# NVlabs/FoundationPose

Measured on NVIDIA H100. Metric: pose-hypotheses/sec at 640x480 RGB-D, 252 hyp, 5 refine iters, higher is better.
Workload: dtype f16

## Files before the change

foundationpose_b200/csrc/fp_api_ops.cu:

```cuda
#include "../../include/fpose.h"
#include "fp_common.cuh"
#include "fp_attn.cuh"
#include "fp_crop.cuh"
#include "fp_gemm.cuh"

#include <vector>

namespace fp {
const char* get_last_error();
int prof_collect(int kind, double* total_ms, double* total_work, int* launches);
}

extern "C" {

const char* fp_last_error(void) { return fp::get_last_error(); }

unsigned long long fp_launch_count(void) { return fp::launch_count(); }

int fp_prof_enable(int on) {
  fp::g_prof_on = on != 0;
  return 0;
}

int fp_prof_collect(int kind, double* total_ms, double* total_work, int* launches) {
  if (!total_ms || !total_work || !launches) {
    fp::set_last_error("fp_prof_collect: null output");
    return -1;
  }
  return fp::prof_collect(kind, total_ms, total_work, launches);
}

int fp_op_build_meshlets(int V, int F, const float* pos, const int* faces, int* info, int* face_of_tri_out,
                         float* meshlets_out) {
  try {
    if (!pos || !faces || !info || V <= 0 || F <= 0) {
      fp::set_last_error("fp_op_build_meshlets: bad argument");
      return -1;
    }
    for (int i = 0; i < 3 * F; ++i)
      if (faces[i] < 0 || faces[i] >= V) {
        fp::set_last_error("fp_op_build_meshlets: face index out of range");
        return -1;
      }
    std::vector<float> nrm((size_t)V * 3, 0.f), att((size_t)V * 3, 0.f);
    fp::MeshHost mh;
    int rc = fp::build_mesh_host(V, F, pos, nrm.data(), att.data(), 3, faces, mh);
    if (rc) return rc;
    int max_t = 0, max_v = 0, total = 0;
    for (const fp::Meshlet& m : mh.meshlets) {
      max_t = m.n_tris > max_t ? m.n_tris : max_t;
      max_v = m.n_verts > max_v ? m.n_verts : max_v;
      total += m.n_tris;
      for (int t = 0; t < m.n_tris; ++t) {
        const uint2 tr = mh.ml_tris[m.tri_off + t];
        for (int k = 0; k < 3; ++k) {
          const int slot = (tr.x >> (8 * k)) & 255;
          if (slot >= m.n_verts || mh.ml_verts[m.vert_off + slot] != faces[3 * tr.y + k]) {
            fp::set_last_error("fp_op_build_meshlets: meshlet triangle does not map back to its face");
            return -4;
          }
          const float* q = pos + 3 * faces[3 * tr.y + k];
          const float dx = q[0] - m.cx, dy = q[1] - m.cy, dz = q[2] - m.cz;
          if (dx * dx + dy * dy + dz * dz > m.r * m.r * 1.0001f + 1e-12f) {
            fp::set_last_error("fp_op_build_meshlets: vertex outside the meshlet's bounding sphere");
            return -4;
          }
        }
        if (face_of_tri_out) face_of_tri_out[m.tri_off + t] = (int)tr.y;
      }
    }
    if (meshlets_out)
      for (size_t i = 0; i < mh.meshlets.size(); ++i) {
        const fp::Meshlet& m = mh.meshlets[i];
        const float rec[8] = {m.cx, m.cy, m.cz, m.r, m.ax, m.ay, m.az, m.cutoff};
        for (int k = 0; k < 8; ++k) meshlets_out[8 * i + k] = rec[k];
      }
    info[0] = (int)mh.meshlets.size();
    info[1] = mh.closed;
    info[2] = mh.front_sign;
    info[3] = max_t;
    info[4] = max_v;
    info[5] = total;
    return 0;
  } catch (...) {
    fp::set_last_error("fp_op_build_meshlets: exception");
    return -3;
  }
}

int fp_op_attention(const void* qkv, void* out, int B, int impl, void* stream) {
  if (!qkv || !out) {
    fp::set_last_error("fp_op_attention: null argument");
    return -1;
  }
  fp::AttnParams ap;
  ap.qkv = reinterpret_cast<const __half*>(qkv);
  ap.ld = 1536;
  ap.q_off = 0;
  ap.k_off = 512;
  ap.v_off = 1024;
  ap.group_col_stride = 0;
  ap.n_groups = 1;
  ap.out = reinterpret_cast<__half*>(out);
  ap.ld_out = 512;
  ap.out_group_stride = 0;
  ap.B = B;
  ap.T = 400;
  ap.n_heads = 4;
  ap.scale = 0.08838834764831845f;
  cudaStream_t st = reinterpret_cast<cudaStream_t>(stream);
  (void)impl;
  return fp::attn_tc_launch(ap, st);
}

static fp::GemmLayer to_gemm_layer(const fp_gemm_layer_t* l) {
  fp::GemmLayer L;
  L.kind = l->kind;
  L.n_img = l->n_img;
  L.Hin = l->Hin;
  L.Win = l->Win;
  L.Cin = l->Cin;
  L.Cout = l->Cout;
  L.in = l->in;
  L.w = l->w;
  L.bias = l->bias;
  L.res = l->res;
  L.res_ld = l->res_ld;
  L.out = l->out;
  L.out_ld = l->out_ld;
  L.out_split = l->out_split;
  L.post_add = l->post_add;
  L.relu = l->relu;
  return L;
}

int fp_op_gemm_layer(const fp_gemm_layer_t* l, void* stream) {
  if (!l) {
    fp::set_last_error("fp_op_gemm_layer: null layer");
    return -1;
  }
  return fp::gemm_layer_launch(to_gemm_layer(l), reinterpret_cast<cudaStream_t>(stream));
}

int fp_op_gemm_tile_n(const fp_gemm_layer_t* l, int* tile_n) {
  if (!l || !tile_n) {
    fp::set_last_error("fp_op_gemm_tile_n: null argument");
    return -1;
  }
  return fp::gemm_layer_tile_n(to_gemm_layer(l), tile_n);
}

}
```

foundationpose_b200/csrc/fp_gemm.cu:

```cuda
#include "fp_gemm.cuh"

#include <stdarg.h>
#include <stdlib.h>
#include <string.h>

#include <mutex>
#include <vector>

#include "fp_common.cuh"
#include "fp_wgmma.cuh"

namespace fp {

static std::atomic<unsigned long long> g_launch_count{0};
static thread_local bool t_capturing = false;
void note_launches(int n) {
  if (!t_capturing) g_launch_count.fetch_add((unsigned long long)n, std::memory_order_relaxed);
}
unsigned long long launch_count() { return g_launch_count.load(std::memory_order_relaxed); }
void set_capturing(bool on) { t_capturing = on; }

std::atomic<bool> g_prof_on{false};
static std::mutex g_prof_mu;

struct ProfRec {
  cudaEvent_t e0, e1;
  double work;
  int kind;
};
static std::vector<ProfRec> g_prof_recs;

void prof_mark_begin(int kind, double work, cudaStream_t stream) {
  if (!g_prof_on) return;
  ProfRec r;
  r.kind = kind;
  r.work = work;
  cudaEventCreate(&r.e0);
  cudaEventCreate(&r.e1);
  cudaEventRecord(r.e0, stream);
  std::lock_guard<std::mutex> lk(g_prof_mu);
  g_prof_recs.push_back(r);
}
void prof_mark_end(cudaStream_t stream) {
  if (!g_prof_on) return;
  std::lock_guard<std::mutex> lk(g_prof_mu);
  if (g_prof_recs.empty()) return;
  cudaEventRecord(g_prof_recs.back().e1, stream);
}
int prof_collect(int kind, double* total_ms, double* total_work, int* launches) {
  FP_CUDA_OK(cudaDeviceSynchronize());
  std::lock_guard<std::mutex> lk(g_prof_mu);
  double ms = 0, work = 0;
  int n = 0;
  std::vector<ProfRec> keep;
  for (auto& r : g_prof_recs) {
    if (r.kind != kind) {
      keep.push_back(r);
      continue;
    }
    float t = 0.f;
    cudaEventElapsedTime(&t, r.e0, r.e1);
    ms += t;
    work += r.work;
    ++n;
    cudaEventDestroy(r.e0);
    cudaEventDestroy(r.e1);
  }
  g_prof_recs.swap(keep);
  *total_ms = ms;
  *total_work = work;
  *launches = n;
  return 0;
}

static thread_local char t_last_error[1024] = "";
void set_last_error(const char* fmt, ...) {
  va_list ap;
  va_start(ap, fmt);
  vsnprintf(t_last_error, sizeof(t_last_error), fmt, ap);
  va_end(ap);
}
const char* get_last_error() { return t_last_error; }

static thread_local int t_pdl_skip = 0;
void pdl_skip_next() { t_pdl_skip = 1; }

bool pdl_enabled() {
  if (t_pdl_skip) {
    t_pdl_skip = 0;
    return false;
  }
  static int on = -1;
  if (on < 0) {
    const char* e = getenv("FPOSE_PDL");
    on = (e && e[0] == '0') ? 0 : 1;
  }
  return on != 0;
}

struct GemmParams {
  int lg_bw, lg_bh;
  int bw, bh, bn;
  int tiles_w, tiles_h, tiles_n, n_tiles_n, total_tiles;
  int num_kb, chunks_per_tap;
  int dim_w, dim_h, dim_n;
  short tap_off[9][5];
  int Ho, Wo, n_img, Cout;
  const float* bias;
  int has_res;
  int odim_h, odim_n;
  int out_split;
  const float* post_add;
  int relu;
  double alg_flops;
};

constexpr int kBlockM = 128;
constexpr int kBlockK = 64;
constexpr int kABytes = kBlockM * kBlockK * 2;
constexpr int kTileThreads = 384;
constexpr int kSlabBytes = kBlockM * 64 * 2;
constexpr int kSmemOptIn = 232448;

constexpr int kWideSlabs = 2;
constexpr int kWideProducerRegs = 40;
constexpr int kWideConsumerRegs = 232;
template <int BN>
struct TileCfg {
  static constexpr int kBBytes = BN * kBlockK * 2;
  static constexpr int kStageBytes = kABytes + kBBytes;
  static constexpr int kSlabs = BN > 128 ? kWideSlabs : BN / 64;
  static constexpr int kPasses = BN / 64 / kSlabs;
  static constexpr int kStagingBytes = kSlabs * kSlabBytes;
  static constexpr int kRing = kSmemOptIn - kStagingBytes - 1024  - 256 ;
  static constexpr int kStages = (kRing / kStageBytes) > 8 ? 8 : (kRing / kStageBytes);
  static constexpr int kSmemBytes = kStages * kStageBytes + kStagingBytes + 1024 + 256;
  static_assert(kSmemBytes <= kSmemOptIn, "tile configuration exceeds the 227 KB opt-in shared memory");
  static_assert(kPasses * kSlabs * 64 == BN, "the epilogue passes must cover the tile's channels");
};

template <int BN>
__global__ void __launch_bounds__(kTileThreads, 1)
    gemm_tile_kernel(const __grid_constant__ CUtensorMap map_a, const __grid_constant__ CUtensorMap map_b,
                     const __grid_constant__ CUtensorMap map_out, const __grid_constant__ CUtensorMap map_res,
                     const __grid_constant__ GemmParams p) {
  using Cfg = TileCfg<BN>;
  constexpr int S = Cfg::kStages;
  constexpr int NSLAB = Cfg::kSlabs;
  constexpr int JP = BN / 8 / Cfg::kPasses;
  extern __shared__ uint8_t smem_raw[];
  uint8_t* smem = reinterpret_cast<uint8_t*>((reinterpret_cast<uintptr_t>(smem_raw) + 1023) & ~uintptr_t(1023));
  uint8_t* staging = smem + S * Cfg::kStageBytes;
  uint64_t* bars = reinterpret_cast<uint64_t*>(staging + Cfg::kStagingBytes);
  uint64_t* full = bars;
  uint64_t* empty = bars + S;
  uint64_t* res_full = bars + 2 * S;

  const int m_tiles = p.tiles_w * p.tiles_h * p.tiles_n;
  const int total = m_tiles * p.n_tiles_n;

  if (threadIdx.x == 0) {
    tma_prefetch_desc(&map_a);
    tma_prefetch_desc(&map_b);
    tma_prefetch_desc(&map_out);
    if (p.has_res) tma_prefetch_desc(&map_res);
    for (int s = 0; s < S; ++s) {
      mbar_init(&full[s], 1);
      mbar_init(&empty[s], 256);
    }
    mbar_init(res_full, 1);
    mbar_fence_init();
  }
  __syncthreads();
  pdl_trigger();
  pdl_wait();

  auto decode = [&](int t, int& n_tile, int& tw, int& th, int& tn) {
    n_tile = t % p.n_tiles_n;
    const int m_tile = t / p.n_tiles_n;
    tw = m_tile % p.tiles_w;
    th = (m_tile / p.tiles_w) % p.tiles_h;
    tn = m_tile / (p.tiles_w * p.tiles_h);
  };

  if (threadIdx.x < 128) {
    if constexpr (BN > 128) regs_release<kWideProducerRegs>();
    if (threadIdx.x == 0) {
      int stage = 0, phase = 0;
      for (int t = blockIdx.x; t < total; t += gridDim.x) {
        int n_tile, tw, th, tn;
        decode(t, n_tile, tw, th, tn);
        int base[5] = {0, 0, 0, 0, 0};
        base[p.dim_w] += tw * p.bw;
        if (p.dim_h >= 0) base[p.dim_h] += th * p.bh;
        if (p.dim_n >= 0) base[p.dim_n] += tn * p.bn;
        int tap = 0, chunk = 0;
        for (int kb = 0; kb < p.num_kb; ++kb) {
          mbar_wait(&empty[stage], phase ^ 1);
          uint8_t* sa = smem + stage * Cfg::kStageBytes;
          mbar_expect_tx(&full[stage], Cfg::kStageBytes);
          tma_load_5d(&map_a, &full[stage], sa, base[0] + p.tap_off[tap][0] + chunk * kBlockK, base[1] + p.tap_off[tap][1],
                      base[2] + p.tap_off[tap][2], base[3] + p.tap_off[tap][3], base[4] + p.tap_off[tap][4]);
          tma_load_2d(&map_b, &full[stage], sa + kABytes, kb * kBlockK, n_tile * BN);
          if (++chunk == p.chunks_per_tap) {
            chunk = 0;
            ++tap;
          }
          if (++stage == S) {
            stage = 0;
            phase ^= 1;
          }
        }
      }
    }
    return;
  }

  if constexpr (BN > 128) regs_acquire<kWideConsumerRegs>();
  const int ct = threadIdx.x - 128;
  const int cw = ct >> 7;
  const int lane = threadIdx.x & 31;
  const int r0 = 64 * cw + 16 * ((ct >> 5) & 3) + (lane >> 2);
  const int cq = 2 * (lane & 3);
  const bool leader = (ct == 0);
  float acc[BN / 2];
#pragma unroll
  for (int i = 0; i < BN / 2; ++i) acc[i] = 0.f;
  int stage = 0, phase = 0, it = 0;
  for (int t = blockIdx.x; t < total; t += gridDim.x, ++it) {
    int n_tile, tw, th, tn;
    decode(t, n_tile, tw, th, tn);
    const int n0 = tn * p.bn;
    int n_o0 = n0, coff = 0;
    if (p.out_split > 0) {
      n_o0 = n0 % p.out_split;
      coff = (n0 / p.out_split) * p.Cout;
    }
    int oc[5] = {0, 0, 0, 0, 0}, rc[5] = {0, 0, 0, 0, 0};
    oc[1] = rc[1] = tw * p.bw;
    if (p.odim_h >= 0) oc[p.odim_h] = rc[p.odim_h] = th * p.bh;
    if (p.odim_n >= 0) {
      oc[p.odim_n] = n_o0;
      rc[p.odim_n] = n0;
    }
    if (leader) asm volatile("cp.async.bulk.wait_group.read 0;" ::: "memory");
    asm volatile("bar.sync 1, 256;" ::: "memory");
    if (leader && p.has_res) {
      mbar_expect_tx(res_full, NSLAB * kSlabBytes);
      for (int s = 0; s < NSLAB; ++s)
        tma_load_5d(&map_res, res_full, staging + s * kSlabBytes, n_tile * BN + s * 64, rc[1], rc[2], rc[3], rc[4]);
    }

    int prev = -1;
    for (int kb = 0; kb < p.num_kb; ++kb) {
      mbar_wait(&full[stage], phase);
      const uint32_t sa = smem_u32(smem + stage * Cfg::kStageBytes);
      const uint64_t da = gmma_desc_sw128(sa + (uint32_t)cw * 8192u);
      const uint64_t db = gmma_desc_sw128(sa + kABytes);
      wgmma_fence();
#pragma unroll
      for (int k = 0; k < kBlockK / 16; ++k)
        Wgmma<BN>::ss(acc, da + (uint64_t)(2 * k), db + (uint64_t)(2 * k), (kb > 0 || k > 0) ? 1u : 0u);
      wgmma_commit();
      if (prev >= 0) {
        wgmma_wait<1>();
        mbar_arrive(&empty[prev]);
      }
      prev = stage;
      if (++stage == S) {
        stage = 0;
        phase ^= 1;
      }
    }
    wgmma_wait<0>();
    fence_regs(acc);
    if (prev >= 0) mbar_arrive(&empty[prev]);

    const float* bias = p.bias + n_tile * BN;
    const float* pap[2] = {nullptr, nullptr};
    if (p.post_add) {
#pragma unroll
      for (int h = 0; h < 2; ++h) {
        const int row = r0 + 8 * h;
        const int jj = row & (p.bw - 1), ii = (row >> p.lg_bw) & (p.bh - 1);
        const int i = th * p.bh + ii, j = min(tw * p.bw + jj, p.Wo - 1);
        pap[h] = p.post_add + (size_t)(i * p.Wo + j) * p.Cout + n_tile * BN;
      }
    }
#pragma unroll
    for (int ps = 0; ps < Cfg::kPasses; ++ps) {
      const int c0 = n_tile * BN + ps * NSLAB * 64;
      if (ps > 0) {
        if (leader) asm volatile("cp.async.bulk.wait_group.read 0;" ::: "memory");
        asm volatile("bar.sync 1, 256;" ::: "memory");
        if (leader && p.has_res) {
          mbar_expect_tx(res_full, NSLAB * kSlabBytes);
          for (int s = 0; s < NSLAB; ++s)
            tma_load_5d(&map_res, res_full, staging + s * kSlabBytes, c0 + s * 64, rc[1], rc[2], rc[3], rc[4]);
        }
      }
      if (p.has_res) mbar_wait(res_full, (uint32_t)((it * Cfg::kPasses + ps) & 1));
#pragma unroll
      for (int jl = 0; jl < JP; ++jl) {
        const int j = ps * JP + jl;
        const int col = 8 * j + cq;
        const float2 b = __ldg(reinterpret_cast<const float2*>(bias + col));
        uint8_t* slab = staging + (jl >> 3) * kSlabBytes;
#pragma unroll
        for (int h = 0; h < 2; ++h) {
          const int row = r0 + 8 * h;
          uint32_t* cell = reinterpret_cast<uint32_t*>(slab + row * 128 + ((((uint32_t)j & 7u) ^ (uint32_t)(row & 7)) << 4) + cq * 2);
          float a0 = acc[4 * j + 2 * h] + b.x, a1 = acc[4 * j + 2 * h + 1] + b.y;
          if (p.has_res) {
            const float2 r = __half22float2(*reinterpret_cast<const __half2*>(cell));
            a0 += r.x;
            a1 += r.y;
          }
          if (p.relu) {
            a0 = fmaxf(a0, 0.f);
            a1 = fmaxf(a1, 0.f);
          }
          if (pap[h]) {
            const float2 pe = __ldg(reinterpret_cast<const float2*>(pap[h] + col));
            a0 += pe.x;
            a1 += pe.y;
          }
          *cell = pack_half2(a0, a1);
        }
      }
      asm volatile("fence.proxy.async.shared::cta;" ::: "memory");
      asm volatile("bar.sync 1, 256;" ::: "memory");
      if (leader) {
        for (int s = 0; s < NSLAB; ++s)
          tma_store_5d(&map_out, staging + s * kSlabBytes, coff + c0 + s * 64, oc[1], oc[2], oc[3], oc[4]);
        asm volatile("cp.async.bulk.commit_group;" ::: "memory");
      }
    }
  }
  if (leader) asm volatile("cp.async.bulk.wait_group 0;" ::: "memory");
}

static int g_num_sms = 0;

typedef CUresult (*EncodeTiledFn)(CUtensorMap*, CUtensorMapDataType, cuuint32_t, void*, const cuuint64_t*,
                                  const cuuint64_t*, const cuuint32_t*, const cuuint32_t*,
                                  CUtensorMapInterleave, CUtensorMapSwizzle, CUtensorMapL2promotion,
                                  CUtensorMapFloatOOBfill);

static EncodeTiledFn get_encode_fn() {
  static EncodeTiledFn fn = nullptr;
  static std::once_flag once;
  std::call_once(once, [] {
    void* p = nullptr;
    cudaDriverEntryPointQueryResult qres;
    if (cudaGetDriverEntryPoint("cuTensorMapEncodeTiled", &p, cudaEnableDefault, &qres) == cudaSuccess &&
        qres == cudaDriverEntryPointSuccess)
      fn = reinterpret_cast<EncodeTiledFn>(p);
  });
  return fn;
}

static int encode_map(CUtensorMap* map, const void* base, int rank, const uint64_t* dims,
                      const uint64_t* strides_bytes , const uint32_t* box, bool swizzle128 = true) {
  EncodeTiledFn fn = get_encode_fn();
  FP_REQUIRE(fn != nullptr, "cuTensorMapEncodeTiled entry point not available (no CUDA driver?)");
  cuuint64_t gdim[5];
  cuuint64_t gstr[4];
  cuuint32_t bdim[5];
  cuuint32_t estr[5];
  for (int i = 0; i < rank; ++i) {
    gdim[i] = dims[i];
    bdim[i] = box[i];
    estr[i] = 1;
  }
  for (int i = 0; i < rank - 1; ++i) gstr[i] = strides_bytes[i];
  CUresult r = fn(map, CU_TENSOR_MAP_DATA_TYPE_FLOAT16, (cuuint32_t)rank, const_cast<void*>(base), gdim, gstr,
                  bdim, estr, CU_TENSOR_MAP_INTERLEAVE_NONE, swizzle128 ? CU_TENSOR_MAP_SWIZZLE_128B : CU_TENSOR_MAP_SWIZZLE_NONE,
                  CU_TENSOR_MAP_L2_PROMOTION_L2_256B, CU_TENSOR_MAP_FLOAT_OOB_FILL_NONE);
  FP_REQUIRE(r == CUDA_SUCCESS,
             "cuTensorMapEncodeTiled failed (%d): rank %d dims [%llu %llu %llu %llu %llu] box [%u %u %u %u %u]",
             (int)r, rank, (unsigned long long)dims[0], (unsigned long long)(rank > 1 ? dims[1] : 0),
             (unsigned long long)(rank > 2 ? dims[2] : 0), (unsigned long long)(rank > 3 ? dims[3] : 0),
             (unsigned long long)(rank > 4 ? dims[4] : 0), box[0], rank > 1 ? box[1] : 0, rank > 2 ? box[2] : 0,
             rank > 3 ? box[3] : 0, rank > 4 ? box[4] : 0);
  return 0;
}

int encode_map_f16(CUtensorMap* map, const void* base, int rank, const uint64_t* dims, const uint64_t* strides_bytes,
                   const uint32_t* box) {
  return encode_map(map, base, rank, dims, strides_bytes, box);
}
int encode_map_f16_linear(CUtensorMap* map, const void* base, int rank, const uint64_t* dims,
                          const uint64_t* strides_bytes, const uint32_t* box) {
  return encode_map(map, base, rank, dims, strides_bytes, box, false);
}
int num_sms() {
  if (g_num_sms == 0) {
    int dev = 0;
    if (cudaGetDevice(&dev) != cudaSuccess) return 0;
    if (cudaDeviceGetAttribute(&g_num_sms, cudaDevAttrMultiProcessorCount, dev) != cudaSuccess) return 0;
  }
  return g_num_sms;
}

static int ilog2(int v) {
  int l = 0;
  while ((1 << l) < v) ++l;
  return l;
}

template <int BN>
static int launch_bn(const CUtensorMap& ma, const CUtensorMap& mb, const CUtensorMap& mo, const CUtensorMap& mr,
                     const GemmParams& p, cudaStream_t stream) {
  using Cfg = TileCfg<BN>;
  static std::atomic<unsigned long long> attr_mask{0};
  if (!device_bit_test(attr_mask)) {
    FP_CUDA_OK(cudaFuncSetAttribute(gemm_tile_kernel<BN>, cudaFuncAttributeMaxDynamicSharedMemorySize, Cfg::kSmemBytes));
    device_bit_set(attr_mask);
  }
  const int sms = num_sms();
  FP_REQUIRE(sms > 0, "no CUDA device");
  const int grid = p.total_tiles < sms ? p.total_tiles : sms;
  prof_mark_begin(0, p.alg_flops, stream);
  FP_CUDA_OK(launch_pdl(gemm_tile_kernel<BN>, dim3(grid), dim3(kTileThreads), Cfg::kSmemBytes, stream, 1, ma, mb, mo, mr, p));
  prof_mark_end(stream);
  note_launches(1);
  FP_CUDA_OK(cudaGetLastError());
  return 0;
}

int stem_conv_launch(const GemmLayer& L, cudaStream_t stream);

static int gemm_layer_plan(const GemmLayer& L, cudaStream_t stream, int* tile_n) {
  if (L.kind == LK_CONV7_S2) {
    if (tile_n) {
      *tile_n = 64;
      return 0;
    }
    return stem_conv_launch(L, stream);
  }
  GemmParams p;
  memset(&p, 0, sizeof(p));
  CUtensorMap ma, mb;
  const uint64_t E = 2;
  int Ho, Wo, taps, ktot;
  int BN;
  uint64_t dims[5], str[4];
  uint32_t box[5];

  switch (L.kind) {
    case LK_LINEAR: {
      FP_REQUIRE(L.Cin % 64 == 0, "LINEAR: K=%d not a multiple of 64", L.Cin);
      Ho = 1;
      Wo = L.Win;
      taps = 1;
      p.chunks_per_tap = L.Cin / 64;
      p.bw = 128; p.bh = 1; p.bn = 1;
      p.dim_w = 1; p.dim_h = -1; p.dim_n = -1;
      dims[0] = L.Cin; dims[1] = L.Win; dims[2] = 1; dims[3] = 1; dims[4] = 1;
      str[0] = L.Cin * E; str[1] = str[0] * L.Win; str[2] = str[1]; str[3] = str[1];
      box[0] = 64; box[1] = 128; box[2] = 1; box[3] = 1; box[4] = 1;
      p.tiles_w = (L.Win + 127) / 128; p.tiles_h = 1; p.tiles_n = 1;
      break;
    }
    case LK_CONV3_S1: {
      FP_REQUIRE(L.Cin % 64 == 0, "CONV3_S1: Cin=%d not a multiple of 64", L.Cin);
      Ho = L.Hin; Wo = L.Win;
      taps = 9;
      p.chunks_per_tap = L.Cin / 64;
      if (Wo % 8 == 0 && Ho % 8 == 0) { p.bw = 8; p.bh = 8; p.bn = 2; }
      else if (Wo % 4 == 0 && Ho % 4 == 0) { p.bw = 4; p.bh = 4; p.bn = 8; }
      else FP_REQUIRE(false, "CONV3_S1: unsupported spatial size %dx%d", Ho, Wo);
      const uint64_t sw_ = (uint64_t)L.Cin * E, sh_ = sw_ * L.Win, sn_ = sh_ * L.Hin;
      p.dim_w = 1; p.dim_h = 2; p.dim_n = 3;
      dims[0] = L.Cin; dims[1] = L.Win; dims[2] = L.Hin; dims[3] = L.n_img; dims[4] = 1;
      str[0] = sw_; str[1] = sh_; str[2] = sn_; str[3] = sn_ * L.n_img;
      box[0] = 64; box[1] = p.bw; box[2] = p.bh; box[3] = p.bn; box[4] = 1;
      for (int r = 0; r < 3; ++r)
        for (int s = 0; s < 3; ++s) {
          p.tap_off[r * 3 + s][1] = (short)(s - 1);
          p.tap_off[r * 3 + s][2] = (short)(r - 1);
        }
      p.tiles_w = Wo / p.bw; p.tiles_h = Ho / p.bh; p.tiles_n = (L.n_img + p.bn - 1) / p.bn;
      break;
    }
    case LK_CONV3_S2: {
      FP_REQUIRE(L.Cin % 64 == 0, "CONV3_S2: Cin=%d not a multiple of 64", L.Cin);
      FP_REQUIRE(L.Hin % 2 == 0 && L.Win % 2 == 0, "CONV3_S2: odd input size");
      Ho = L.Hin / 2; Wo = L.Win / 2;
      taps = 9;
      p.chunks_per_tap = L.Cin / 64;
      if (Wo % 8 == 0 && Ho % 8 == 0) { p.bw = 8; p.bh = 8; p.bn = 2; }
      else if (Wo % 4 == 0 && Ho % 4 == 0) { p.bw = 4; p.bh = 4; p.bn = 8; }
      else FP_REQUIRE(false, "CONV3_S2: unsupported output size %dx%d", Ho, Wo);
      p.dim_w = 1; p.dim_h = 3; p.dim_n = 4;
      dims[0] = 2 * L.Cin; dims[1] = Wo; dims[2] = 2; dims[3] = Ho; dims[4] = L.n_img;
      str[0] = 2 * L.Cin * E; str[1] = (uint64_t)L.Win * L.Cin * E; str[2] = 2 * str[1];
      str[3] = (uint64_t)L.Hin * L.Win * L.Cin * E;
      box[0] = 64; box[1] = p.bw; box[2] = 1; box[3] = p.bh; box[4] = p.bn;
      for (int r = 0; r < 3; ++r)
        for (int s = 0; s < 3; ++s) {
          const int t = r * 3 + s;
          p.tap_off[t][0] = (short)((s == 1 ? 0 : 1) * L.Cin);
          p.tap_off[t][1] = (short)(s == 0 ? -1 : 0);
          p.tap_off[t][2] = (short)(r == 1 ? 0 : 1);
          p.tap_off[t][3] = (short)(r == 0 ? -1 : 0);
        }
      p.tiles_w = Wo / p.bw; p.tiles_h = Ho / p.bh; p.tiles_n = (L.n_img + p.bn - 1) / p.bn;
      break;
    }
    default:
      FP_REQUIRE(false, "unknown layer kind %d", L.kind);
  }
  ktot = taps * L.Cin;
  p.num_kb = ktot / 64;
  p.lg_bw = ilog2(p.bw);
  p.lg_bh = ilog2(p.bh);

  constexpr int kWideMinWaves = 8;
  constexpr int kWideMinKBlocks = 16;
  const int m_tiles = p.tiles_w * p.tiles_h * p.tiles_n;
  if (L.Cout % 256 == 0 && p.num_kb >= kWideMinKBlocks) {
    const int sms = num_sms();
    FP_REQUIRE(sms > 0, "no CUDA device");
    BN = (long long)m_tiles * (L.Cout / 256) >= (long long)kWideMinWaves * sms ? 256 : 128;
  } else if (L.Cout % 128 == 0) BN = 128;
  else if (L.Cout % 64 == 0) BN = 64;
  else FP_REQUIRE(false, "Cout=%d must be a multiple of 64", L.Cout);
  p.n_tiles_n = L.Cout / BN;
  p.total_tiles = p.tiles_w * p.tiles_h * p.tiles_n * p.n_tiles_n;
  p.Ho = Ho; p.Wo = Wo; p.n_img = L.n_img; p.Cout = L.Cout;
  p.bias = L.bias;
  p.has_res = L.res != nullptr;
  p.out_split = L.out_split;
  p.post_add = L.post_add;
  p.relu = L.relu;
  {
    const double k_real = (double)taps * L.Cin;
    p.alg_flops = 2.0 * (double)L.n_img * Ho * Wo * L.Cout * k_real;
  }
  FP_REQUIRE(L.out_ld % 8 == 0 && (!L.res || L.res_ld % 8 == 0), "out_ld / res_ld must be multiples of 8");
  FP_REQUIRE(L.out_split == 0 || L.out_split % p.bn == 0,
             "out_split=%d must be a multiple of the tile's image count %d (pad the A/B batch boundary)", L.out_split,
             p.bn);
  if (tile_n) {
    *tile_n = BN;
    return 0;
  }
  if (p.total_tiles == 0) return 0;

  int rc = encode_map(&ma, L.in, 5, dims, str, box);
  if (rc) return rc;
  uint64_t wd[2] = {(uint64_t)ktot, (uint64_t)L.Cout};
  uint64_t ws[1] = {(uint64_t)ktot * E};
  uint32_t wb[2] = {64, (uint32_t)BN};
  rc = encode_map(&mb, L.w, 2, wd, ws, wb);
  if (rc) return rc;
  CUtensorMap mo, mr;
  {
    uint64_t od[5], os[4];
    uint32_t ob[5];
    const bool lin = (L.kind == LK_LINEAR);
    const int n_out = L.out_split > 0 ? (L.n_img - L.out_split) : L.n_img;
    FP_REQUIRE(n_out > 0, "out_split=%d leaves no output images (n_img=%d)", L.out_split, L.n_img);
    auto fill = [&](int ld, int nimg) {
      const uint64_t sw_ = (uint64_t)ld * E, sh_ = sw_ * Wo, sn_ = sh_ * Ho;
      od[0] = (uint64_t)ld;
      ob[0] = 64;
      od[4] = 1;
      ob[4] = 1;
      if (lin) {
        od[1] = (uint64_t)Wo; od[2] = 1; od[3] = 1;
        os[0] = sw_; os[1] = sh_; os[2] = sh_; os[3] = sh_;
        ob[1] = (uint32_t)p.bw; ob[2] = 1; ob[3] = 1;
      } else {
        od[1] = (uint64_t)Wo; od[2] = (uint64_t)Ho; od[3] = (uint64_t)nimg;
        os[0] = sw_; os[1] = sh_; os[2] = sn_; os[3] = sn_ * nimg;
        ob[1] = (uint32_t)p.bw; ob[2] = (uint32_t)p.bh; ob[3] = (uint32_t)p.bn;
      }
    };
    p.odim_h = lin ? -1 : 2;
    p.odim_n = lin ? -1 : 3;
    fill(L.out_ld, n_out);
    rc = encode_map(&mo, L.out, 5, od, os, ob);
    if (rc) return rc;
    if (L.res) {
      fill(L.res_ld, L.n_img);
      rc = encode_map(&mr, L.res, 5, od, os, ob);
      if (rc) return rc;
    } else {
      mr = mo;
    }
  }
  if (BN == 256) return launch_bn<256>(ma, mb, mo, mr, p, stream);
  return BN == 128 ? launch_bn<128>(ma, mb, mo, mr, p, stream) : launch_bn<64>(ma, mb, mo, mr, p, stream);
}

int gemm_layer_launch(const GemmLayer& L, cudaStream_t stream) { return gemm_layer_plan(L, stream, nullptr); }

int gemm_layer_tile_n(const GemmLayer& L, int* tile_n) { return gemm_layer_plan(L, nullptr, tile_n); }

}
```

foundationpose_b200/csrc/fp_gemm.cuh:

```cuda
#pragma once
#include <cuda.h>
#include <cuda_runtime.h>
#include <stdint.h>

#include <atomic>

namespace fp {

enum LayerKind : int {
  LK_LINEAR = 0,
  LK_CONV3_S1 = 1,
  LK_CONV3_S2 = 2,
  LK_CONV7_S2 = 3,
};

struct GemmLayer {
  int kind;
  int n_img;
  int Hin, Win;
  int Cin;
  int Cout;
  const void* in;
  const void* w;
  const float* bias;
  const void* res;
  int res_ld;
  void* out;
  int out_ld;
  int out_split;
  const float* post_add;
  int relu;
};

int gemm_layer_launch(const GemmLayer& L, cudaStream_t stream);
int gemm_layer_tile_n(const GemmLayer& L, int* tile_n);


void prof_mark_begin(int kind, double work, cudaStream_t stream);
void prof_mark_end(cudaStream_t stream);
extern std::atomic<bool> g_prof_on;

}
```

foundationpose_b200/ops.py:

```python
import ctypes as C

import torch

from . import _lib
from ._lib import lib


def _ptr(t):
    return None if t is None else C.c_void_p(t.data_ptr())


def _stream():
    return C.c_void_p(torch.cuda.current_stream().cuda_stream)


def _require_cuda(*ts):
    for t in ts:
        if t is not None and not t.is_cuda:
            raise _lib.FposeError("libfpose operators need CUDA tensors (there is no CPU path)")


def gemm_layer(kind, x, w_packed, bias, *, n_img, Hin, Win, Cin, Cout, out=None, out_ld=None, out_split=0,
               res=None, res_ld=0, post_add=None, relu=False):
    _require_cuda(x, w_packed, bias, res, post_add, out)
    assert x.dtype == torch.float16 and w_packed.dtype == torch.float16 and bias.dtype == torch.float32
    if kind == _lib.LAYER_LINEAR:
        Ho, Wo = 1, Win
    elif kind == _lib.LAYER_CONV3_S1:
        Ho, Wo = Hin, Win
    else:
        Ho, Wo = Hin // 2, Win // 2
    if out is None:
        out_ld = Cout
        out = torch.empty(n_img, Ho, Wo, Cout, dtype=torch.float16, device=x.device)
    L = _lib.GemmLayer(kind, n_img, Hin, Win, Cin, Cout, _ptr(x), _ptr(w_packed), _ptr(bias), _ptr(res),
                       res_ld, _ptr(out), out_ld, out_split, _ptr(post_add), 1 if relu else 0)
    _lib.check(lib.fp_op_gemm_layer(C.byref(L), _stream()), "fp_op_gemm_layer")
    return out


def gemm_tile_n(kind, *, n_img, Hin, Win, Cin, Cout, out_split=0):
    lib.fp_op_gemm_tile_n.argtypes = [C.POINTER(_lib.GemmLayer), C.POINTER(C.c_int)]
    lib.fp_op_gemm_tile_n.restype = C.c_int
    L = _lib.GemmLayer(kind, n_img, Hin, Win, Cin, Cout, None, None, None, None, 0, None, Cout, out_split, None, 0)
    tile_n = C.c_int(0)
    _lib.check(lib.fp_op_gemm_tile_n(C.byref(L), C.byref(tile_n)), "fp_op_gemm_tile_n")
    return tile_n.value


lib.fp_op_attention.argtypes = [C.c_void_p, C.c_void_p, C.c_int, C.c_int, C.c_void_p]
lib.fp_op_attention.restype = C.c_int


def attention(qkv, impl=1):
    _require_cuda(qkv)
    assert qkv.dtype == torch.float16 and qkv.shape[1] == 1536 and qkv.shape[0] % 400 == 0
    B = qkv.shape[0] // 400
    out = torch.empty(qkv.shape[0], 512, dtype=torch.float16, device=qkv.device)
    _lib.check(lib.fp_op_attention(_ptr(qkv), _ptr(out), B, impl, _stream()), "fp_op_attention")
    return out
```

include/fpose.h:

```cpp
#ifndef FPOSE_H_
#define FPOSE_H_

#include <stddef.h>
#include <stdint.h>

#ifdef __cplusplus
extern "C" {
#endif

const char* fp_last_error(void);
unsigned long long fp_launch_count(void);

int fp_prof_enable(int on);
int fp_prof_collect(int kind, double* total_ms, double* total_work, int* launches);


#define FP_LAYER_LINEAR 0
#define FP_LAYER_CONV3_S1 1
#define FP_LAYER_CONV3_S2 2
#define FP_LAYER_CONV7_S2 3

typedef struct fp_gemm_layer {
  int kind;
  int n_img;
  int Hin, Win;
  int Cin;
  int Cout;
  const void* in;
  const void* w;
  const float* bias;
  const void* res;
  int res_ld;
  void* out;
  int out_ld;
  int out_split;
  const float* post_add;
  int relu;
} fp_gemm_layer_t;

int fp_op_gemm_layer(const fp_gemm_layer_t* layer, void* stream);
int fp_op_gemm_tile_n(const fp_gemm_layer_t* layer, int* tile_n);

int fp_op_attention(const void* qkv, void* out, int B, int impl, void* stream);


typedef struct fp_ctx fp_ctx;

int fp_create(fp_ctx** ctx);
int fp_destroy(fp_ctx* ctx);

int fp_set_config(fp_ctx* ctx, int which, float crop_ratio, float rot_normalizer);

typedef struct fp_tensor {
  const char* name;
  const void* data;
  int dtype;
  long long numel;
} fp_tensor_t;

int fp_load_network(fp_ctx* ctx, int which, const fp_tensor_t* tensors, int n);

int fp_set_mesh(fp_ctx* ctx, int V, int F, const float* pos, const float* nrm, const float* uv, const float* vcol,
                const int* faces, const unsigned char* tex_rgb, int Ht, int Wt, float diameter);
#define FP_MAX_MESHES 64
int fp_set_mesh_slot(fp_ctx* ctx, int slot, int V, int F, const float* pos, const float* nrm, const float* uv,
                     const float* vcol, const int* faces, const unsigned char* tex_rgb, int Ht, int Wt, float diameter);
int fp_mesh_info(fp_ctx* ctx, int* info);

#define FP_FRAME_ON_DEVICE 1
#define FP_FRAME_FILTER_DEPTH 2
int fp_set_frame(fp_ctx* ctx, const unsigned char* rgb, const float* depth, const float* K, int H, int W, int flags,
                 float zfar, void* stream);
int fp_set_xyz_map(fp_ctx* ctx, const float* xyz, void* stream);
int fp_get_depth(fp_ctx* ctx, float* depth_out_dev, float* xyz_out_dev, void* stream);

int fp_start_poses(fp_ctx* ctx, const unsigned char* mask, int mask_on_device, const float* rot_grid, int N,
                   float* poses_out, float* info_out, void* stream);

int fp_make_crops(fp_ctx* ctx, const float* poses, int N, int mode, void* crops_out, float* dbg_out, float* win_out,
                  void* stream);
int fp_set_crop_tile(fp_ctx* ctx, int tile);
int fp_crop_stats(fp_ctx* ctx, const float* poses, int N, int mode, int* stats_out_host, void* stream);

int fp_refine(fp_ctx* ctx, const float* poses_in, int N, int iterations, float* poses_out, float* last_trans,
              float* last_rot, void* stream);

int fp_score(fp_ctx* ctx, const float* poses, int N, float* scores_out, int* best_out, void* stream);
int fp_score_features(fp_ctx* ctx, const float* poses, int N, float* feats_out, void* stream);
int fp_score_tail(fp_ctx* ctx, const float* feats, int L, float* scores_out, int* best_out, void* stream);

int fp_register(fp_ctx* ctx, const float* poses_host, int N, int iterations, float* poses_out_host,
                float* scores_out_host, int* best_out_host, void* stream);

int fp_track(fp_ctx* ctx, const unsigned char* rgb_host, const float* depth_host, const float* K, int H, int W,
             const float* pose_in_dev, int iterations, float* pose_out_dev, float* pose_out_host, void* stream);
int fp_track_objects(fp_ctx* ctx, const unsigned char* rgb_host, const float* depth_host, const float* K, int H, int W,
                     int M, const int* slots_host, const float* poses_in_dev, int iterations, float* poses_out_dev,
                     float* poses_out_host, void* stream);
#define FP_MAX_CAMERAS 16
int fp_track_cameras(fp_ctx* ctx, int C, const unsigned char* const* rgb_host, const float* const* depth_host,
                     const float* K, const int* H, const int* W, int M, const int* camera_of, const int* slots_host,
                     const float* poses_in_dev, int iterations, float* poses_out_dev, float* poses_out_host, void* stream);
int fp_register_objects(fp_ctx* ctx, const unsigned char* rgb_host, const float* depth_host, const float* K, int H, int W,
                        int M, const int* slots_host, const int* n_hyp_host, const unsigned char* masks_host,
                        const float* rot_grids_dev, int iterations, float* poses_out_dev, float* scores_out_dev,
                        int* best_out_dev, float* info_out_dev, void* stream);
int fp_register_cameras(fp_ctx* ctx, int C, const unsigned char* const* rgb_host, const float* const* depth_host,
                        const float* K, const int* H, const int* W, int M, const int* camera_of, const int* slots_host,
                        const int* n_hyp_host, const unsigned char* const* masks_host, const float* rot_grids_dev,
                        int iterations, float* poses_out_dev, float* scores_out_dev, int* best_out_dev, float* info_out_dev,
                        void* stream);
unsigned long long fp_graph_captures(fp_ctx* ctx);

typedef struct fp_group fp_group;
int fp_group_create(int ndev, const int* dev_ids, fp_group** out);
int fp_group_destroy(fp_group* g);
int fp_group_size(fp_group* g);
fp_ctx* fp_group_ctx(fp_group* g, int i);
int fp_group_load_network(fp_group* g, int which, const fp_tensor_t* tensors, int n);
int fp_group_set_config(fp_group* g, int which, float crop_ratio, float rot_normalizer);
int fp_group_set_mesh(fp_group* g, int V, int F, const float* pos, const float* nrm, const float* uv, const float* vcol,
                      const int* faces, const unsigned char* tex_rgb, int Ht, int Wt, float diameter);
int fp_group_register(fp_group* g, const unsigned char* rgb_host, const float* depth_host, const float* K, int H, int W,
                      const unsigned char* mask_host, const float* rot_grid_host, int N, int iterations,
                      float* poses_out_host, float* scores_out_host, int* best_out_host, float* info_out_host);

int fp_op_refine_net(fp_ctx* ctx, const void* crops, int N, float* trans_out, float* rot_out, void* stream);
int fp_op_score_feats(fp_ctx* ctx, const void* crops, int N, float* feats_out, void* stream);
int fp_op_tokens(fp_ctx* ctx, int which, const void* crops, int N, void* tokens_out, void* stream);
int fp_op_build_meshlets(int V, int F, const float* pos, const int* faces, int* info, int* face_of_tri_out,
                         float* meshlets_out );
int fp_op_depth_filter(const float* depth_dev, float* out_dev, int H, int W, int which, void* stream);
int fp_op_pose_update(const float* poses_in, const float* trans, const float* rot, float* poses_out, int N,
                      float mesh_diameter, float rot_normalizer, void* stream);

#ifdef __cplusplus
}
#endif
#endif
```

Baseline: 2641.

## Add ping-pong warpgroup schedule for 128-wide GEMM tiles

Adds a ping-pong variant of the warp-specialized GEMM kernel for 128-wide tiles. Each consumer warpgroup owns a whole 128x128 tile, and the two warpgroups alternate tiles using named barriers, so one group's epilogue overlaps the other's MMA mainloop. It is selected automatically when there are at least twice as many tiles as SMs. Staging shared memory is doubled, which cuts the ring to 5 stages, and register reallocation is enabled for the larger per-warpgroup accumulator. This adds barrier-ordering complexity and a risk of bank or stage-phase mistakes.

After: 2670 (median of 6 runs). 1.01x the previous value.

```diff
diff --git a/foundationpose_b200/csrc/fp_api_ops.cu b/foundationpose_b200/csrc/fp_api_ops.cu
--- a/foundationpose_b200/csrc/fp_api_ops.cu
+++ b/foundationpose_b200/csrc/fp_api_ops.cu
@@ -142,12 +142,29 @@
   return fp::gemm_layer_launch(to_gemm_layer(l), reinterpret_cast<cudaStream_t>(stream));
 }
 
-int fp_op_gemm_tile_n(const fp_gemm_layer_t* l, int* tile_n) {
-  if (!l || !tile_n) {
-    fp::set_last_error("fp_op_gemm_tile_n: null argument");
+int fp_op_gemm_layer_schedule(const fp_gemm_layer_t* l, int schedule, void* stream) {
+  if (!l) {
+    fp::set_last_error("fp_op_gemm_layer_schedule: null layer");
     return -1;
   }
-  return fp::gemm_layer_tile_n(to_gemm_layer(l), tile_n);
+  if (schedule != FP_GEMM_COOPERATIVE && schedule != FP_GEMM_PINGPONG) {
+    fp::set_last_error("fp_op_gemm_layer_schedule: unknown schedule %d", schedule);
+    return -1;
+  }
+  return fp::gemm_layer_launch(to_gemm_layer(l), reinterpret_cast<cudaStream_t>(stream), schedule);
+}
+
+int fp_op_gemm_tile_n(const fp_gemm_layer_t* l, int* tile_n) {
+  int schedule = 0;
+  return fp_op_gemm_tile_config(l, tile_n, &schedule);
+}
+
+int fp_op_gemm_tile_config(const fp_gemm_layer_t* l, int* tile_n, int* schedule) {
+  if (!l || !tile_n || !schedule) {
+    fp::set_last_error("fp_op_gemm_tile_config: null argument");
+    return -1;
+  }
+  return fp::gemm_layer_tile_config(to_gemm_layer(l), tile_n, schedule);
 }
 
 }
diff --git a/foundationpose_b200/csrc/fp_gemm.cu b/foundationpose_b200/csrc/fp_gemm.cu
--- a/foundationpose_b200/csrc/fp_gemm.cu
+++ b/foundationpose_b200/csrc/fp_gemm.cu
@@ -125,29 +125,33 @@
 constexpr int kWideSlabs = 2;
 constexpr int kWideProducerRegs = 40;
 constexpr int kWideConsumerRegs = 232;
-template <int BN>
+
+template <int BN, bool PP>
 struct TileCfg {
   static constexpr int kBBytes = BN * kBlockK * 2;
   static constexpr int kStageBytes = kABytes + kBBytes;
   static constexpr int kSlabs = BN > 128 ? kWideSlabs : BN / 64;
   static constexpr int kPasses = BN / 64 / kSlabs;
-  static constexpr int kStagingBytes = kSlabs * kSlabBytes;
+  static constexpr int kStagingBytes = (PP ? 2 : 1) * kSlabs * kSlabBytes;
   static constexpr int kRing = kSmemOptIn - kStagingBytes - 1024  - 256 ;
   static constexpr int kStages = (kRing / kStageBytes) > 8 ? 8 : (kRing / kStageBytes);
   static constexpr int kSmemBytes = kStages * kStageBytes + kStagingBytes + 1024 + 256;
   static_assert(kSmemBytes <= kSmemOptIn, "tile configuration exceeds the 227 KB opt-in shared memory");
   static_assert(kPasses * kSlabs * 64 == BN, "the epilogue passes must cover the tile's channels");
+  static_assert(!PP || (BN == 128 && kStages == 5), "ping-pong: 128-wide tiles, 64 KB of staging beside 5 stages");
 };
 
-template <int BN>
+template <int BN, bool PP>
 __global__ void __launch_bounds__(kTileThreads, 1)
     gemm_tile_kernel(const __grid_constant__ CUtensorMap map_a, const __grid_constant__ CUtensorMap map_b,
                      const __grid_constant__ CUtensorMap map_out, const __grid_constant__ CUtensorMap map_res,
                      const __grid_constant__ GemmParams p) {
-  using Cfg = TileCfg<BN>;
+  using Cfg = TileCfg<BN, PP>;
   constexpr int S = Cfg::kStages;
   constexpr int NSLAB = Cfg::kSlabs;
   constexpr int JP = BN / 8 / Cfg::kPasses;
+  constexpr int NH = PP ? 2 : 1;
+  constexpr bool kRealloc = BN > 128 || PP;
   extern __shared__ uint8_t smem_raw[];
   uint8_t* smem = reinterpret_cast<uint8_t*>((reinterpret_cast<uintptr_t>(smem_raw) + 1023) & ~uintptr_t(1023));
   uint8_t* staging = smem + S * Cfg::kStageBytes;
@@ -166,9 +170,10 @@
     if (p.has_res) tma_prefetch_desc(&map_res);
     for (int s = 0; s < S; ++s) {
       mbar_init(&full[s], 1);
-      mbar_init(&empty[s], 256);
+      mbar_init(&empty[s], PP ? 128 : 256);
     }
     mbar_init(res_full, 1);
+    if (PP) mbar_init(res_full + 1, 1);
     mbar_fence_init();
   }
   __syncthreads();
@@ -184,7 +189,7 @@
   };
 
   if (threadIdx.x < 128) {
-    if constexpr (BN > 128) regs_release<kWideProducerRegs>();
+    if constexpr (kRealloc) regs_release<kWideProducerRegs>();
     if (threadIdx.x == 0) {
       int stage = 0, phase = 0;
       for (int t = blockIdx.x; t < total; t += gridDim.x) {
@@ -216,18 +221,33 @@
     return;
   }
 
-  if constexpr (BN > 128) regs_acquire<kWideConsumerRegs>();
+  if constexpr (kRealloc) regs_acquire<kWideConsumerRegs>();
   const int ct = threadIdx.x - 128;
   const int cw = ct >> 7;
   const int lane = threadIdx.x & 31;
-  const int r0 = 64 * cw + 16 * ((ct >> 5) & 3) + (lane >> 2);
+  const int r0 = (PP ? 0 : 64 * cw) + 16 * ((ct >> 5) & 3) + (lane >> 2);
   const int cq = 2 * (lane & 3);
-  const bool leader = (ct == 0);
-  float acc[BN / 2];
-#pragma unroll
-  for (int i = 0; i < BN / 2; ++i) acc[i] = 0.f;
+  const bool leader = PP ? (ct & 127) == 0 : ct == 0;
+  if constexpr (PP) {
+    staging += cw * NSLAB * kSlabBytes;
+    res_full += cw;
+  }
+  auto staging_sync = [&] {
+    if constexpr (PP) asm volatile("bar.sync %0, 128;" ::"r"(1 + cw) : "memory");
+    else asm volatile("bar.sync 1, 256;" ::: "memory");
+  };
+  float acc[NH][BN / 2];
+#pragma unroll
+  for (int hv = 0; hv < NH; ++hv)
+#pragma unroll
+    for (int i = 0; i < BN / 2; ++i) acc[hv][i] = 0.f;
   int stage = 0, phase = 0, it = 0;
-  for (int t = blockIdx.x; t < total; t += gridDim.x, ++it) {
+  for (int t = blockIdx.x + (PP ? cw * (int)gridDim.x : 0); t < total; t += (PP ? 2 : 1) * gridDim.x, ++it) {
+    if constexpr (PP) {
+      const int g = (2 * it + cw) * p.num_kb;
+      stage = g % S;
+      phase = (g / S) & 1;
+    }
     int n_tile, tw, th, tn;
     decode(t, n_tile, tw, th, tn);
     const int n0 = tn * p.bn;
@@ -244,23 +264,27 @@
       rc[p.odim_n] = n0;
     }
     if (leader) asm volatile("cp.async.bulk.wait_group.read 0;" ::: "memory");
-    asm volatile("bar.sync 1, 256;" ::: "memory");
+    staging_sync();
     if (leader && p.has_res) {
       mbar_expect_tx(res_full, NSLAB * kSlabBytes);
       for (int s = 0; s < NSLAB; ++s)
         tma_load_5d(&map_res, res_full, staging + s * kSlabBytes, n_tile * BN + s * 64, rc[1], rc[2], rc[3], rc[4]);
     }
+    if constexpr (PP)
+      if (t != (int)blockIdx.x) asm volatile("bar.sync %0, 256;" ::"r"(3 + cw) : "memory");
 
     int prev = -1;
     for (int kb = 0; kb < p.num_kb; ++kb) {
       mbar_wait(&full[stage], phase);
       const uint32_t sa = smem_u32(smem + stage * Cfg::kStageBytes);
-      const uint64_t da = gmma_desc_sw128(sa + (uint32_t)cw * 8192u);
+      const uint64_t da = gmma_desc_sw128(sa + (uint32_t)(PP ? 0 : cw) * 8192u);
       const uint64_t db = gmma_desc_sw128(sa + kABytes);
       wgmma_fence();
 #pragma unroll
       for (int k = 0; k < kBlockK / 16; ++k)
-        Wgmma<BN>::ss(acc, da + (uint64_t)(2 * k), db + (uint64_t)(2 * k), (kb > 0 || k > 0) ? 1u : 0u);
+#pragma unroll
+        for (int hv = 0; hv < NH; ++hv)
+          Wgmma<BN>::ss(acc[hv], da + (uint64_t)(512 * hv + 2 * k), db + (uint64_t)(2 * k), (kb > 0 || k > 0) ? 1u : 0u);
       wgmma_commit();
       if (prev >= 0) {
         wgmma_wait<1>();
@@ -272,27 +296,32 @@
         phase ^= 1;
       }
     }
+    if constexpr (PP)
+      if (t + (int)gridDim.x < total) asm volatile("bar.arrive %0, 256;" ::"r"(3 + (cw ^ 1)) : "memory");
     wgmma_wait<0>();
-    fence_regs(acc);
+#pragma unroll
+    for (int hv = 0; hv < NH; ++hv) fence_regs(acc[hv]);
     if (prev >= 0) mbar_arrive(&empty[prev]);
 
     const float* bias = p.bias + n_tile * BN;
-    const float* pap[2] = {nullptr, nullptr};
+    const float* pap[NH][2] = {};
     if (p.post_add) {
 #pragma unroll
-      for (int h = 0; h < 2; ++h) {
-        const int row = r0 + 8 * h;
-        const int jj = row & (p.bw - 1), ii = (row >> p.lg_bw) & (p.bh - 1);
-        const int i = th * p.bh + ii, j = min(tw * p.bw + jj, p.Wo - 1);
-        pap[h] = p.post_add + (size_t)(i * p.Wo + j) * p.Cout + n_tile * BN;
-      }
+      for (int hv = 0; hv < NH; ++hv)
+#pragma unroll
+        for (int h = 0; h < 2; ++h) {
+          const int row = r0 + 64 * hv + 8 * h;
+          const int jj = row & (p.bw - 1), ii = (row >> p.lg_bw) & (p.bh - 1);
+          const int i = th * p.bh + ii, j = min(tw * p.bw + jj, p.Wo - 1);
+          pap[hv][h] = p.post_add + (size_t)(i * p.Wo + j) * p.Cout + n_tile * BN;
+        }
     }
 #pragma unroll
     for (int ps = 0; ps < Cfg::kPasses; ++ps) {
       const int c0 = n_tile * BN + ps * NSLAB * 64;
       if (ps > 0) {
         if (leader) asm volatile("cp.async.bulk.wait_group.read 0;" ::: "memory");
-        asm volatile("bar.sync 1, 256;" ::: "memory");
+        staging_sync();
         if (leader && p.has_res) {
           mbar_expect_tx(res_full, NSLAB * kSlabBytes);
           for (int s = 0; s < NSLAB; ++s)
@@ -307,29 +336,31 @@
         const float2 b = __ldg(reinterpret_cast<const float2*>(bias + col));
         uint8_t* slab = staging + (jl >> 3) * kSlabBytes;
 #pragma unroll
-        for (int h = 0; h < 2; ++h) {
-          const int row = r0 + 8 * h;
-          uint32_t* cell = reinterpret_cast<uint32_t*>(slab + row * 128 + ((((uint32_t)j & 7u) ^ (uint32_t)(row & 7)) << 4) + cq * 2);
-          float a0 = acc[4 * j + 2 * h] + b.x, a1 = acc[4 * j + 2 * h + 1] + b.y;
-          if (p.has_res) {
-            const float2 r = __half22float2(*reinterpret_cast<const __half2*>(cell));
-            a0 += r.x;
-            a1 += r.y;
+        for (int hv = 0; hv < NH; ++hv)
+#pragma unroll
+          for (int h = 0; h < 2; ++h) {
+            const int row = r0 + 64 * hv + 8 * h;
+            uint32_t* cell = reinterpret_cast<uint32_t*>(slab + row * 128 + ((((uint32_t)j & 7u) ^ (uint32_t)(row & 7)) << 4) + cq * 2);
+            float a0 = acc[hv][4 * j + 2 * h] + b.x, a1 = acc[hv][4 * j + 2 * h + 1] + b.y;
+            if (p.has_res) {
+              const float2 r = __half22float2(*reinterpret_cast<const __half2*>(cell));
+              a0 += r.x;
+              a1 += r.y;
+            }
+            if (p.relu) {
+              a0 = fmaxf(a0, 0.f);
+              a1 = fmaxf(a1, 0.f);
+            }
+            if (pap[hv][h]) {
+              const float2 pe = __ldg(reinterpret_cast<const float2*>(pap[hv][h] + col));
+              a0 += pe.x;
+              a1 += pe.y;
+            }
+            *cell = pack_half2(a0, a1);
           }
-          if (p.relu) {
-            a0 = fmaxf(a0, 0.f);
-            a1 = fmaxf(a1, 0.f);
-          }
-          if (pap[h]) {
-            const float2 pe = __ldg(reinterpret_cast<const float2*>(pap[h] + col));
-            a0 += pe.x;
-            a1 += pe.y;
-          }
-          *cell = pack_half2(a0, a1);
-        }
       }
       asm volatile("fence.proxy.async.shared::cta;" ::: "memory");
-      asm volatile("bar.sync 1, 256;" ::: "memory");
+      staging_sync();
       if (leader) {
         for (int s = 0; s < NSLAB; ++s)
           tma_store_5d(&map_out, staging + s * kSlabBytes, coff + c0 + s * 64, oc[1], oc[2], oc[3], oc[4]);
@@ -409,20 +440,20 @@
   return l;
 }
 
-template <int BN>
+template <int BN, bool PP = false>
 static int launch_bn(const CUtensorMap& ma, const CUtensorMap& mb, const CUtensorMap& mo, const CUtensorMap& mr,
                      const GemmParams& p, cudaStream_t stream) {
-  using Cfg = TileCfg<BN>;
+  using Cfg = TileCfg<BN, PP>;
   static std::atomic<unsigned long long> attr_mask{0};
   if (!device_bit_test(attr_mask)) {
-    FP_CUDA_OK(cudaFuncSetAttribute(gemm_tile_kernel<BN>, cudaFuncAttributeMaxDynamicSharedMemorySize, Cfg::kSmemBytes));
+    FP_CUDA_OK(cudaFuncSetAttribute(gemm_tile_kernel<BN, PP>, cudaFuncAttributeMaxDynamicSharedMemorySize, Cfg::kSmemBytes));
     device_bit_set(attr_mask);
   }
   const int sms = num_sms();
   FP_REQUIRE(sms > 0, "no CUDA device");
   const int grid = p.total_tiles < sms ? p.total_tiles : sms;
   prof_mark_begin(0, p.alg_flops, stream);
-  FP_CUDA_OK(launch_pdl(gemm_tile_kernel<BN>, dim3(grid), dim3(kTileThreads), Cfg::kSmemBytes, stream, 1, ma, mb, mo, mr, p));
+  FP_CUDA_OK(launch_pdl(gemm_tile_kernel<BN, PP>, dim3(grid), dim3(kTileThreads), Cfg::kSmemBytes, stream, 1, ma, mb, mo, mr, p));
   prof_mark_end(stream);
   note_launches(1);
   FP_CUDA_OK(cudaGetLastError());
@@ -431,10 +462,13 @@
 
 int stem_conv_launch(const GemmLayer& L, cudaStream_t stream);
 
-static int gemm_layer_plan(const GemmLayer& L, cudaStream_t stream, int* tile_n) {
+static int gemm_layer_plan(const GemmLayer& L, cudaStream_t stream, int force, int* tile_n, int* sched) {
+  FP_REQUIRE(force == GS_AUTO || force == GS_COOPERATIVE || force == GS_PINGPONG, "unknown GEMM schedule %d", force);
   if (L.kind == LK_CONV7_S2) {
+    FP_REQUIRE(force != GS_PINGPONG, "the stem convolution has no ping-pong schedule");
     if (tile_n) {
       *tile_n = 64;
+      *sched = GS_COOPERATIVE;
       return 0;
     }
     return stem_conv_launch(L, stream);
@@ -529,6 +563,16 @@
   else FP_REQUIRE(false, "Cout=%d must be a multiple of 64", L.Cout);
   p.n_tiles_n = L.Cout / BN;
   p.total_tiles = p.tiles_w * p.tiles_h * p.tiles_n * p.n_tiles_n;
+  int schedule = GS_COOPERATIVE;
+  if (BN == 128 && L.kind != LK_CONV3_S2) {
+    const int sms = num_sms();
+    FP_REQUIRE(sms > 0, "no CUDA device");
+    schedule = p.total_tiles >= 2 * sms ? GS_PINGPONG : GS_COOPERATIVE;
+  }
+  if (force != GS_AUTO) {
+    FP_REQUIRE(force == GS_COOPERATIVE || BN == 128, "the %d-wide tile has no ping-pong schedule", BN);
+    schedule = force;
+  }
   p.Ho = Ho; p.Wo = Wo; p.n_img = L.n_img; p.Cout = L.Cout;
   p.bias = L.bias;
   p.has_res = L.res != nullptr;
@@ -545,6 +589,7 @@
              p.bn);
   if (tile_n) {
     *tile_n = BN;
+    *sched = schedule;
     return 0;
   }
   if (p.total_tiles == 0) return 0;
@@ -593,11 +638,18 @@
     }
   }
   if (BN == 256) return launch_bn<256>(ma, mb, mo, mr, p, stream);
-  return BN == 128 ? launch_bn<128>(ma, mb, mo, mr, p, stream) : launch_bn<64>(ma, mb, mo, mr, p, stream);
-}
-
-int gemm_layer_launch(const GemmLayer& L, cudaStream_t stream) { return gemm_layer_plan(L, stream, nullptr); }
-
-int gemm_layer_tile_n(const GemmLayer& L, int* tile_n) { return gemm_layer_plan(L, nullptr, tile_n); }
-
-}
+  if (BN == 128)
+    return schedule == GS_PINGPONG ? launch_bn<128, true>(ma, mb, mo, mr, p, stream)
+                                   : launch_bn<128>(ma, mb, mo, mr, p, stream);
+  return launch_bn<64>(ma, mb, mo, mr, p, stream);
+}
+
+int gemm_layer_launch(const GemmLayer& L, cudaStream_t stream, int schedule) {
+  return gemm_layer_plan(L, stream, schedule, nullptr, nullptr);
+}
+
+int gemm_layer_tile_config(const GemmLayer& L, int* tile_n, int* schedule) {
+  return gemm_layer_plan(L, nullptr, GS_AUTO, tile_n, schedule);
+}
+
+}
diff --git a/foundationpose_b200/csrc/fp_gemm.cuh b/foundationpose_b200/csrc/fp_gemm.cuh
--- a/foundationpose_b200/csrc/fp_gemm.cuh
+++ b/foundationpose_b200/csrc/fp_gemm.cuh
@@ -32,8 +32,10 @@
   int relu;
 };
 
-int gemm_layer_launch(const GemmLayer& L, cudaStream_t stream);
-int gemm_layer_tile_n(const GemmLayer& L, int* tile_n);
+enum GemmSchedule : int { GS_AUTO = -1, GS_COOPERATIVE = 0, GS_PINGPONG = 1 };
+
+int gemm_layer_launch(const GemmLayer& L, cudaStream_t stream, int schedule = GS_AUTO);
+int gemm_layer_tile_config(const GemmLayer& L, int* tile_n, int* schedule);
 
 
 void prof_mark_begin(int kind, double work, cudaStream_t stream);
diff --git a/foundationpose_b200/ops.py b/foundationpose_b200/ops.py
--- a/foundationpose_b200/ops.py
+++ b/foundationpose_b200/ops.py
@@ -20,8 +20,11 @@
             raise _lib.FposeError("libfpose operators need CUDA tensors (there is no CPU path)")
 
 
+COOPERATIVE, PINGPONG = 0, 1
+
+
 def gemm_layer(kind, x, w_packed, bias, *, n_img, Hin, Win, Cin, Cout, out=None, out_ld=None, out_split=0,
-               res=None, res_ld=0, post_add=None, relu=False):
+               res=None, res_ld=0, post_add=None, relu=False, schedule=None):
     _require_cuda(x, w_packed, bias, res, post_add, out)
     assert x.dtype == torch.float16 and w_packed.dtype == torch.float16 and bias.dtype == torch.float32
     if kind == _lib.LAYER_LINEAR:
@@ -35,17 +38,26 @@
         out = torch.empty(n_img, Ho, Wo, Cout, dtype=torch.float16, device=x.device)
     L = _lib.GemmLayer(kind, n_img, Hin, Win, Cin, Cout, _ptr(x), _ptr(w_packed), _ptr(bias), _ptr(res),
                        res_ld, _ptr(out), out_ld, out_split, _ptr(post_add), 1 if relu else 0)
-    _lib.check(lib.fp_op_gemm_layer(C.byref(L), _stream()), "fp_op_gemm_layer")
+    if schedule is None:
+        _lib.check(lib.fp_op_gemm_layer(C.byref(L), _stream()), "fp_op_gemm_layer")
+    else:
+        lib.fp_op_gemm_layer_schedule.argtypes = [C.POINTER(_lib.GemmLayer), C.c_int, C.c_void_p]
+        lib.fp_op_gemm_layer_schedule.restype = C.c_int
+        _lib.check(lib.fp_op_gemm_layer_schedule(C.byref(L), schedule, _stream()), "fp_op_gemm_layer_schedule")
     return out
 
 
 def gemm_tile_n(kind, *, n_img, Hin, Win, Cin, Cout, out_split=0):
-    lib.fp_op_gemm_tile_n.argtypes = [C.POINTER(_lib.GemmLayer), C.POINTER(C.c_int)]
-    lib.fp_op_gemm_tile_n.restype = C.c_int
+    return gemm_tile_config(kind, n_img=n_img, Hin=Hin, Win=Win, Cin=Cin, Cout=Cout, out_split=out_split)[0]
+
+
+def gemm_tile_config(kind, *, n_img, Hin, Win, Cin, Cout, out_split=0):
+    lib.fp_op_gemm_tile_config.argtypes = [C.POINTER(_lib.GemmLayer), C.POINTER(C.c_int), C.POINTER(C.c_int)]
+    lib.fp_op_gemm_tile_config.restype = C.c_int
     L = _lib.GemmLayer(kind, n_img, Hin, Win, Cin, Cout, None, None, None, None, 0, None, Cout, out_split, None, 0)
-    tile_n = C.c_int(0)
-    _lib.check(lib.fp_op_gemm_tile_n(C.byref(L), C.byref(tile_n)), "fp_op_gemm_tile_n")
-    return tile_n.value
+    tile_n, schedule = C.c_int(0), C.c_int(0)
+    _lib.check(lib.fp_op_gemm_tile_config(C.byref(L), C.byref(tile_n), C.byref(schedule)), "fp_op_gemm_tile_config")
+    return tile_n.value, schedule.value
 
 
 lib.fp_op_attention.argtypes = [C.c_void_p, C.c_void_p, C.c_int, C.c_int, C.c_void_p]
diff --git a/include/fpose.h b/include/fpose.h
--- a/include/fpose.h
+++ b/include/fpose.h
@@ -40,6 +40,11 @@
 
 int fp_op_gemm_layer(const fp_gemm_layer_t* layer, void* stream);
 int fp_op_gemm_tile_n(const fp_gemm_layer_t* layer, int* tile_n);
+
+#define FP_GEMM_COOPERATIVE 0
+#define FP_GEMM_PINGPONG 1
+int fp_op_gemm_tile_config(const fp_gemm_layer_t* layer, int* tile_n, int* schedule);
+int fp_op_gemm_layer_schedule(const fp_gemm_layer_t* layer, int schedule, void* stream);
 
 int fp_op_attention(const void* qkv, void* out, int B, int impl, void* stream);
 
```
